# jpe17/TwoTowerMLRetrieval

Measured on AMD Instinct MI355X. Metric: queries/sec top-k over 10M x 256-d docs, higher is better.
Workload: dtype f32 results (bit-identical to the fp32 FMA chain); f16-MFMA screen + fp32 rescoring; 1 GPU; exact cosine top-10 of B=1024 queries over 10000000 x 256 fp32 unit-norm passages resident in HBM (BASELINE configs[3]; configs[1] batch), row-sharded over 1 GPU(s), screened path (f16-MFMA filter + exact fp32 rescoring, bit-identical to the fp32 kernel); n_docs=10000000, dim=256, batch=1024, k=10, parallelism=rowshard1

## Files before the change

### twotowermlretrieval_amd/csrc/screen.hip

```cpp
#include "score_topk.h"
#include "keep_word.h"
#include <cmath>

#include <hip/hip_fp16.h>
#include <limits.h>
#include <math.h>

namespace {

typedef _Float16 h8 __attribute__((ext_vector_type(8)));
typedef _Float16 h4 __attribute__((ext_vector_type(4)));
typedef unsigned u32x4 __attribute__((ext_vector_type(4)));
typedef __attribute__((address_space(3))) void lds_void;
typedef const __attribute__((address_space(1))) void gbl_void;

#ifndef TT_SCREEN_STAGGER
#define TT_SCREEN_STAGGER 1
#endif
constexpr int SW = 8;
constexpr int STILE_BYTES = 32 * 512;
constexpr int SRING = 8;
constexpr int STPB = 2;
constexpr int SCAP = 128;
constexpr int SURV_MAX = 1024;
constexpr int POOL_MAX = 8192;
constexpr int FIN_MAX_CHUNKS = 2048;

struct SCand {
    float v;
    int x;
};

__device__ __forceinline__ float screen_eps(float qnorm, float dmax)
{
    return 1.10e-3f * qnorm * dmax + 1e-6f * (qnorm + dmax);
}

template <int NCH>
__device__ __forceinline__ void bf16_to_f16_lds(char *base, int lane)
{
    uint4 v[NCH];
#pragma unroll
    for (int i = 0; i < NCH; ++i)
        v[i] = *(const uint4 *)(base + (i * 64 + lane) * 16);
#pragma unroll
    for (int i = 0; i < NCH; ++i) {
        unsigned w[4] = {v[i].x, v[i].y, v[i].z, v[i].w};
#pragma unroll
        for (int e = 0; e < 4; ++e) {
            const _Float16 lo = (_Float16)__uint_as_float(w[e] << 16);
            const _Float16 hi = (_Float16)__uint_as_float(w[e] & 0xffff0000u);
            w[e] = (unsigned)__builtin_bit_cast(unsigned short, lo) | ((unsigned)__builtin_bit_cast(unsigned short, hi) << 16);
        }
        *(uint4 *)(base + (i * 64 + lane) * 16) = uint4{w[0], w[1], w[2], w[3]};
    }
}

__device__ __forceinline__ SCand scand_load_l2(const SCand *p)
{
    unsigned long long u = __hip_atomic_load((const unsigned long long *)p, __ATOMIC_RELAXED, __HIP_MEMORY_SCOPE_AGENT);
    SCand c;
    c.v = __uint_as_float((unsigned)u);
    c.x = (int)(u >> 32);
    return c;
}

struct ScreenParams {
    const float *Q;
    const _Float16 *D16;
    int B, N, k;
    int n_chunks, tiles_per_chunk, n_tiles;
    int static_tiles, tail_g, tail_blocks;
    int *tail_ctr;
    float dmax;
    SCand *cand;
    int *pcnt;
    int *flag;
    float *max_val;
    const float *thr0;
    int thr0_stride;
    const h8 *qimg;
    const float *qnorm;
    const float *dbg_thr;
    const unsigned *keep;
};

__device__ __forceinline__ void scand_store_async(const SCand *base, unsigned byte_off, float v, int x)
{
    const unsigned long long bits = ((unsigned long long)(unsigned)x << 32) | (unsigned long long)__float_as_uint(v);
    asm volatile("global_store_dwordx2 %0, %1, %2\n\ts_nop 1" ::"v"(byte_off), "v"(bits), "s"(base) : "memory");
}

__device__ __forceinline__ void f32_store_async(float *dst, float v)
{
    asm volatile("global_store_dword %0, %1, off\n\ts_nop 0" ::"v"(dst), "v"(v) : "memory");
}

constexpr int SQUART = SCAP / 4;
constexpr int SQ_TRIGGER = SQUART - 10;
constexpr int SQ_KEEP_MAX = 4 * SQ_TRIGGER - 4;

__device__ __forceinline__ void screen_compact(SCand *base, const int (&n)[4], int k, float slack, int lane, int &n_new,
                                               float &thr_new, bool &have, bool &overflow)
{
    float v[2];
    int x[2], rank[2];
    bool live[2];
#pragma unroll
    for (int i = 0; i < 2; ++i) {
        v[i] = -INFINITY;
        x[i] = INT_MAX;
        rank[i] = 0;
        live[i] = (lane & 31) < ((lane >> 5) ? n[2 * i + 1] : n[2 * i]);
        if (live[i]) {
            const SCand c = scand_load_l2(base + 64 * i + lane);
            v[i] = c.v;
            x[i] = c.x;
        }
    }
#pragma unroll
    for (int i2 = 0; i2 < 2; ++i2) {
#pragma unroll
        for (int sub = 0; sub < 2; ++sub) {
            const int lim = n[2 * i2 + sub];
            for (int l2 = 0; l2 < lim; ++l2) {
                const float sv = __builtin_bit_cast(float, __builtin_amdgcn_readlane(__builtin_bit_cast(int, v[i2]), 32 * sub + l2));
                const int sx = __builtin_amdgcn_readlane(x[i2], 32 * sub + l2);
#pragma unroll
                for (int i = 0; i < 2; ++i)
                    rank[i] += (sv > v[i] || (sv == v[i] && sx < x[i])) ? 1 : 0;
            }
        }
    }
    const int total = n[0] + n[1] + n[2] + n[3];
    have = total >= k;
    overflow = false;
    n_new = total;
    thr_new = -INFINITY;
    if (have) {
        float kth = -INFINITY;
#pragma unroll
        for (int i = 0; i < 2; ++i) {
            const unsigned long long bk = __ballot(live[i] && rank[i] == k - 1);
            if (bk)
                kth = __builtin_bit_cast(float, __builtin_amdgcn_readlane(__builtin_bit_cast(int, v[i]), __ffsll((long long)bk) - 1));
        }
        thr_new = kth - slack;
        n_new = 0;
#pragma unroll
        for (int i = 0; i < 2; ++i)
            n_new += __popcll(__ballot(live[i] && v[i] >= thr_new));
        if (n_new > SQ_KEEP_MAX) {
            overflow = true;
            n_new = k;
        }
    }
#pragma unroll
    for (int i = 0; i < 2; ++i)
        if (live[i] && rank[i] < n_new) {
            SCand c;
            c.v = v[i];
            c.x = x[i];
            base[SQUART * (rank[i] & 3) + (rank[i] >> 2)] = c;
        }
}

__global__ __launch_bounds__(128) void q_image_kernel(const float *__restrict__ Q, int B, h8 *__restrict__ img,
                                                      float *__restrict__ qnorm, int *__restrict__ flag, int n_flags,
                                                      int *__restrict__ tail_ctr, int n_ctr)
{
    __shared__ int any_bad[2];
    if (blockIdx.x == 0)
        for (int i = threadIdx.x; i < n_ctr; i += 128)
            tail_ctr[i] = 0;
    const int lane = threadIdx.x & 63, wv = threadIdx.x >> 6;
    const int S = blockIdx.x * 2 + wv;
    const int g = lane >> 4, n = lane & 15;
    const int qrow = 16 * S + n;
    const bool live = qrow < B;
    const float *qp = Q + (size_t)min(qrow, B - 1) * 256 + 8 * g;
    float ss = 0.0f;
    bool bad = false;
#pragma unroll
    for (int s = 0; s < 8; ++s) {
        const f32x4 a = *(const f32x4 *)(qp + 32 * s);
        const f32x4 b = *(const f32x4 *)(qp + 32 * s + 4);
        h8 hv;
#pragma unroll
        for (int e = 0; e < 4; ++e) {
            const float x0 = live ? a[e] : 0.0f, x1 = live ? b[e] : 0.0f;
            ss += x0 * x0 + x1 * x1;
            bad |= !(fabsf(x0) <= 60000.0f) || !(fabsf(x1) <= 60000.0f);
            hv[e] = (_Float16)x0;
            hv[4 + e] = (_Float16)x1;
        }
        img[((size_t)S * 8 + s) * 64 + lane] = hv;
    }
    ss += __shfl_xor(ss, 16);
    ss += __shfl_xor(ss, 32);
    if (g == 0)
        qnorm[qrow] = sqrtf(ss);
    const bool wave_bad = __ballot(bad && live) != 0ull;
    if (lane == 0)
        any_bad[wv] = wave_bad ? 1 : 0;
    __syncthreads();
    if (threadIdx.x == 0 && (int)blockIdx.x < n_flags)
        flag[blockIdx.x] = (any_bad[0] | any_bad[1]) ? 2 : 0;
}

template <bool MAXONLY, int NSET, bool BF = false, bool MASKED = false>
__global__ __launch_bounds__(SW * 64, 2) void screen_kernel(ScreenParams p)
{
    extern __shared__ __attribute__((aligned(16))) char ring[];
    constexpr int DMA_AUX = NSET < 3 ? 2 : 0;
    const int lane = threadIdx.x & 63;
    const int w = __builtin_amdgcn_readfirstlane(threadIdx.x >> 6);
    const int chunk = blockIdx.x % p.n_chunks;
    const int qgroup = blockIdx.x / p.n_chunks;
    int t0 = chunk * p.tiles_per_chunk;
    int t1 = min(t0 + p.tiles_per_chunk, p.static_tiles);
    __shared__ int next_block;
    const int k = p.k;
    const int g = lane >> 4, n = lane & 15;
    constexpr int QW = 16 * NSET, QB = SW * QW;
    const int qbase = qgroup * QB + w * QW;
    const bool wave_live = qbase < p.B;

    h8 qreg[NSET][8];
    float eps2[NSET];
    f32x4 negthr[NSET];
    int cnt[NSET];
#pragma unroll
    for (int c = 0; c < NSET; ++c)
        cnt[c] = 0;
#pragma unroll
    for (int c = 0; c < NSET; ++c) {
        const int qrow = qbase + 16 * c + n;
        const bool live = qrow < p.B;
        float qn = 0.0f;
        if (wave_live) {
            const h8 *src = p.qimg + ((size_t)(qbase / 16 + c) * 8) * 64 + lane;
#pragma unroll
            for (int s = 0; s < 8; ++s)
                qreg[c][s] = src[s * 64];
            qn = p.qnorm[qrow];
        }
        eps2[c] = 2.0f * screen_eps(qn, p.dmax);
        const float floor_thr = -(1.01f * qn * p.dmax + 1e-30f);
        const float t_init = live ? ((!MAXONLY && p.thr0) ? fmaxf(p.thr0[(size_t)qrow * p.thr0_stride + p.thr0_stride - 1] - eps2[c], floor_thr)
                                                    : floor_thr)
                            : INFINITY;
        float c_init = -t_init;
        if (MAXONLY)
            c_init = (p.dbg_thr && live) ? -p.dbg_thr[qrow] : 0.0f;
        negthr[c] = f32x4{c_init, c_init, c_init, c_init};
    }

    SCand *const cwave = p.cand + ((size_t)blockIdx.x * QB + w * QW) * SCAP;

    auto compact_where = [&](int c, unsigned qmask) {
        asm volatile("s_waitcnt vmcnt(0)" ::: "memory");
        while (qmask) {
            const int q = __ffs((int)qmask) - 1;
            qmask &= qmask - 1;
            const int nq[4] = {__builtin_amdgcn_readlane(cnt[c], q), __builtin_amdgcn_readlane(cnt[c], q + 16),
                               __builtin_amdgcn_readlane(cnt[c], q + 32), __builtin_amdgcn_readlane(cnt[c], q + 48)};
            const float slack = __builtin_bit_cast(float, __builtin_amdgcn_readlane(__builtin_bit_cast(int, eps2[c]), q));
            int n_new;
            float tn;
            bool have, ovf;
            screen_compact(cwave + (size_t)(16 * c + q) * SCAP, nq, k, slack, lane, n_new, tn, have, ovf);
            if (ovf && lane == 0)
                atomicOr(p.flag + ((qbase + 16 * c) >> 5), 1);
            if (n == q) {
                cnt[c] = (n_new - g + 3) >> 2;
                if (have)
                    negthr[c] = f32x4{-tn, -tn, -tn, -tn};
            }
        }
    };

    const char *D = (const char *)p.D16;
    const char *rowp[2];
    auto set_rows = [&](int tile) {
#pragma unroll
        for (int i = 0; i < 2; ++i) {
            const int row = 2 * (2 * w + i) + (lane >> 5);
            const int doc = min(tile * 32 + row, p.N - 1);
            const int chunk16 = (lane & 31) ^ (row & 15);
            rowp[i] = D + (size_t)doc * 512 + chunk16 * 16;
        }
    };
    auto dma_issue = [&](int tile, int stage) {
        set_rows(min(tile, t1 - 1));
        char *dst = ring + stage * STILE_BYTES + (2 * w) * 1024;
        __builtin_amdgcn_global_load_lds((gbl_void *)rowp[0], (lds_void *)dst, 16, 0, DMA_AUX);
        __builtin_amdgcn_global_load_lds((gbl_void *)rowp[1], (lds_void *)(dst + 1024), 16, 0, DMA_AUX);
    };
    auto dma_piece = [&](int i, int stage) {
        char *dst = ring + stage * STILE_BYTES + (2 * w + i) * 1024;
        __builtin_amdgcn_global_load_lds((gbl_void *)rowp[i], (lds_void *)dst, 16, 0, DMA_AUX);
    };

    for (;;) {
    if (t0 < t1) {
#pragma unroll
        for (int gi = 0; gi < SRING - STPB; ++gi)
            dma_issue(t0 + gi, gi);
        int stage = 0;
        const int rd_base = n * 512;
        f32x4 acc[2][NSET];
        const bool late = TT_SCREEN_STAGGER && w >= 4;
        bool pending = false;
        int ptile = 0;
        unsigned pkw = 0xffffffffu;
        auto epilogue = [&](int tile, unsigned kw) {
                const int tile_base = tile * 32;
            const bool partial = tile_base + 32 > p.N;
            const bool holes = MASKED && kw != 0xffffffffu;
            const unsigned kwg = MASKED ? kw >> (4 * g) : 0xffffffffu;
            auto dropped = [&](int u, int r) {
                return tile_base + 16 * u + 4 * g + r >= p.N || (MASKED && ((kwg >> (16 * u + r)) & 1u) == 0u);
            };
            if (!MAXONLY) {
                if (partial || holes) {
#pragma unroll
                    for (int u = 0; u < 2; ++u)
#pragma unroll
                        for (int r = 0; r < 4; ++r)
                            if (dropped(u, r)) {
#pragma unroll
                                for (int c = 0; c < NSET; ++c)
                                    acc[u][c][r] = -INFINITY;
                            }
                }
                int mall = INT_MIN;
#pragma unroll
                for (int u = 0; u < 2; ++u)
#pragma unroll
                    for (int c = 0; c < NSET; ++c)
#pragma unroll
                        for (int r = 0; r < 4; ++r)
                            mall = max(mall, __float_as_int(acc[u][c][r]));
                if (__ballot(mall >= 0) != 0ull) {
#pragma unroll
                    for (int c = 0; c < NSET; ++c) {
                        int mu[2];
#pragma unroll
                        for (int u = 0; u < 2; ++u)
                            mu[u] = max(max(__float_as_int(acc[u][c][0]), __float_as_int(acc[u][c][1])),
                                        max(__float_as_int(acc[u][c][2]), __float_as_int(acc[u][c][3])));
                        if (__ballot(max(mu[0], mu[1]) >= 0) == 0ull)
                            continue;
                        const unsigned mine = (unsigned)(((16 * c + n) * SCAP + SQUART * g) * sizeof(SCand));
                        const float thr_c = -negthr[c][0];
#pragma unroll
                        for (int u = 0; u < 2; ++u) {
                            if (__ballot(mu[u] >= 0) == 0ull)
                                continue;
#pragma unroll
                            for (int r = 0; r < 4; ++r) {
                                if (__float_as_int(acc[u][c][r]) >= 0) {
                                    scand_store_async(cwave, mine + (unsigned)cnt[c] * (unsigned)sizeof(SCand),
                                                      acc[u][c][r] + thr_c, tile_base + 16 * u + 4 * g + r);
                                    ++cnt[c];
                                }
                            }
                        }
                        unsigned long long full = __ballot(cnt[c] > SQ_TRIGGER);
                        full = (full | (full >> 32));
                        full = (full | (full >> 16)) & 0xffffull;
                        if (full)
                            compact_where(c, (unsigned)full);
                    }
                }
            } else {
#pragma unroll
                for (int c = 0; c < NSET; ++c) {
                    float m = -INFINITY;
                    if (!partial && !holes) {
                        int mi = INT_MIN;
#pragma unroll
                        for (int u = 0; u < 2; ++u)
#pragma unroll
                            for (int r = 0; r < 4; ++r)
                                mi = max(mi, __float_as_int(acc[u][c][r]));
                        m = __int_as_float(mi);
                    } else {
#pragma unroll
                        for (int u = 0; u < 2; ++u)
#pragma unroll
                            for (int r = 0; r < 4; ++r)
                                m = fmaxf(m, !dropped(u, r) ? acc[u][c][r] : -INFINITY);
                    }
                    m = fmaxf(m, __shfl_xor(m, 16));
                    m = fmaxf(m, __shfl_xor(m, 32));
                    const int qrow = qbase + 16 * c + n;
                    if (g == 0 && qrow < p.B)
                        f32_store_async(p.max_val + (size_t)qrow * p.n_tiles + tile, m);
                }
            }
                };
        for (int tile = t0; tile < t1; ++tile) {
            if ((tile - t0) % STPB == 0) {
                asm volatile("s_waitcnt vmcnt(%0)" ::"n"(2 * (SRING - 2 * STPB)) : "memory");
                if (BF && tile == t0) {
#pragma unroll
                    for (int i = 0; i < STPB; ++i)
                        bf16_to_f16_lds<2>(ring + ((stage + i) % SRING) * STILE_BYTES + (2 * w) * 1024, lane);
                    asm volatile("s_waitcnt lgkmcnt(0)" ::: "memory");
                }
                __builtin_amdgcn_s_barrier();
            } else if (BF && (tile - t0) % STPB == STPB - 1) {
                asm volatile("s_waitcnt vmcnt(%0)" ::"n"(2 * (SRING - 3 * STPB + 1)) : "memory");
#pragma unroll
                for (int i = 1; i <= STPB; ++i)
                    bf16_to_f16_lds<2>(ring + ((stage + i) % SRING) * STILE_BYTES + (2 * w) * 1024, lane);
                asm volatile("s_waitcnt lgkmcnt(0)" ::: "memory");
            }
            const int fill_stage = (stage + SRING - STPB) % SRING;
            set_rows(min(tile + SRING - STPB, t1 - 1));
            if (!wave_live) {
                dma_piece(0, fill_stage);
                dma_piece(1, fill_stage);
            }
            if (wave_live) {
                if (late && pending)
                    epilogue(ptile, pkw);
                const char *buf = ring + stage * STILE_BYTES + rd_base;
                h8 a0[3], a1[3];
                auto a_read = [&](int s) {
                    const int off = ((4 * s + g) ^ n) << 4;
                    a0[s % 3] = *(const h8 *)(buf + off);
                    a1[s % 3] = *(const h8 *)(buf + 16 * 512 + off);
                };
                a_read(0);
                a_read(1);
                unsigned kw = 0xffffffffu;
#pragma unroll
                for (int s = 0; s < 8; ++s) {
                    if (s + 2 < 8)
                        a_read(s + 2);
                    if (MASKED && s == 0)
                        keep_word_issue(p.keep + __builtin_amdgcn_readfirstlane(tile), kw, a0[0]);
                    if (s == 2)
                        dma_piece(0, fill_stage);
                    if (s == 6)
                        dma_piece(1, fill_stage);
                    __builtin_amdgcn_sched_barrier(0);
#pragma unroll
                    for (int c = 0; c < NSET; ++c) {
                        const f32x4 c0 = s == 0 ? negthr[c] : acc[0][c];
                        const f32x4 c1 = s == 0 ? negthr[c] : acc[1][c];
                        acc[0][c] = __builtin_amdgcn_mfma_f32_16x16x32_f16(a0[s % 3], qreg[c][s], c0, 0, 0, 0);
                        acc[1][c] = __builtin_amdgcn_mfma_f32_16x16x32_f16(a1[s % 3], qreg[c][s], c1, 0, 0, 0);
                    }
                    __builtin_amdgcn_sched_barrier(0);
                }
                if (MASKED)
                    keep_word_wait(kw, acc[1][NSET - 1]);
                if (late) {
                    pending = true;
                    ptile = tile;
                    pkw = kw;
                } else {
                    epilogue(tile, kw);
                }
            }
            stage = (stage + 1) % SRING;
        }
        if (wave_live && late && pending)
            epilogue(ptile, pkw);
    }
    if (MAXONLY || p.tail_blocks == 0)
        break;
    asm volatile("s_waitcnt vmcnt(0)" ::: "memory");
    __builtin_amdgcn_s_barrier();
    if (threadIdx.x == 0)
        next_block = atomicAdd(p.tail_ctr + qgroup, 1);
    __syncthreads();
    const int blk = next_block;
    if (blk >= p.tail_blocks)
        break;
    t0 = p.static_tiles + blk * p.tail_g;
    t1 = min(t0 + p.tail_g, p.n_tiles);
    }
    asm volatile("s_waitcnt vmcnt(0)" ::: "memory");
    __builtin_amdgcn_s_barrier();

    if (MAXONLY)
        return;
#pragma unroll
    for (int c = 0; c < NSET; ++c) {
        int tot = cnt[c] + __shfl_xor(cnt[c], 16);
        tot += __shfl_xor(tot, 32);
        const unsigned long long over = __ballot(tot > k) & 0xffffull;
        if (over)
            compact_where(c, (unsigned)over);
        int packed = cnt[c] << (8 * g);
        packed |= __shfl_xor(packed, 16);
        packed |= __shfl_xor(packed, 32);
        const int qrow = qbase + 16 * c + n;
        if (g == 0 && qrow < p.B)
            p.pcnt[(size_t)qrow * p.n_chunks + chunk] = packed;
    }
}

constexpr int TW = 4;
constexpr int TSLAB_BYTES = 32 * 128;
constexpr int TSTAGE = 4;
constexpr int TDMA = 4;
constexpr int TSTREAM_AUX = 2;

template <bool MAXONLY, int NQS = 2, bool BF = false, bool MASKED = false>
__global__ __launch_bounds__(TW * 64, 2) void screen_stream_kernel(ScreenParams p)
{
    constexpr int QPT = 16 * NQS;
    extern __shared__ __attribute__((aligned(16))) char ring_all[];
    const int lane = threadIdx.x & 63;
    const int w = __builtin_amdgcn_readfirstlane(threadIdx.x >> 6);
    char *const ring = ring_all + w * (TSTAGE * TSLAB_BYTES);
    const int task = blockIdx.x * TW + w;
    const int n_qtiles = (p.B + QPT - 1) / QPT;
    if (task >= n_qtiles * p.n_chunks)
        return;
    const int qtile = task / p.n_chunks, chunk = task % p.n_chunks;
    const int t0 = chunk * p.tiles_per_chunk;
    const int t1 = min(t0 + p.tiles_per_chunk, p.n_tiles);
    const int k = p.k;
    const int g = lane >> 4, n = lane & 15;
    const int qbase = qtile * QPT;

    h8 qreg[NQS][8];
    float eps2[NQS];
    f32x4 negthr[NQS];
    int cnt[NQS];
#pragma unroll
    for (int c = 0; c < NQS; ++c) {
        cnt[c] = 0;
        const int qrow = qbase + 16 * c + n;
        const bool live = qrow < p.B;
        const h8 *src = p.qimg + ((size_t)(qbase / 16 + c) * 8) * 64 + lane;
#pragma unroll
        for (int s = 0; s < 8; ++s)
            qreg[c][s] = src[s * 64];
        const float qn = p.qnorm[qrow];
        eps2[c] = 2.0f * screen_eps(qn, p.dmax);
        const float floor_thr = -(1.01f * qn * p.dmax + 1e-30f);
        const float t_init = live ? ((!MAXONLY && p.thr0) ? fmaxf(p.thr0[(size_t)qrow * p.thr0_stride + p.thr0_stride - 1] - eps2[c], floor_thr)
                                                    : floor_thr)
                            : INFINITY;
        float c_init = -t_init;
        if (MAXONLY)
            c_init = (p.dbg_thr && live) ? -p.dbg_thr[qrow] : 0.0f;
        negthr[c] = f32x4{c_init, c_init, c_init, c_init};
    }

    SCand *const cwave = p.cand + (size_t)task * QPT * SCAP;

    auto compact_where = [&](int c, unsigned qmask) {
        asm volatile("s_waitcnt vmcnt(0)" ::: "memory");
        while (qmask) {
            const int q = __ffs((int)qmask) - 1;
            qmask &= qmask - 1;
            const int nq[4] = {__builtin_amdgcn_readlane(cnt[c], q), __builtin_amdgcn_readlane(cnt[c], q + 16),
                               __builtin_amdgcn_readlane(cnt[c], q + 32), __builtin_amdgcn_readlane(cnt[c], q + 48)};
            const float slack = __builtin_bit_cast(float, __builtin_amdgcn_readlane(__builtin_bit_cast(int, eps2[c]), q));
            int n_new;
            float tn;
            bool have, ovf;
            screen_compact(cwave + (size_t)(16 * c + q) * SCAP, nq, k, slack, lane, n_new, tn, have, ovf);
            if (ovf && lane == 0)
                atomicOr(p.flag + ((qbase + 16 * c) >> 5), 1);
            if (n == q) {
                cnt[c] = (n_new - g + 3) >> 2;
                if (have)
                    negthr[c] = f32x4{-tn, -tn, -tn, -tn};
            }
        }
    };

    const char *D = (const char *)p.D16;
    int dma_tile = t0, dma_kq = 0;
    const char *rowp[TDMA];
    auto set_rows = [&](int tile) {
#pragma unroll
        for (int jj = 0; jj < TDMA; ++jj) {
            const int row = 8 * jj + (lane >> 3);
            const int doc = min(tile * 32 + row, p.N - 1);
            rowp[jj] = D + (size_t)doc * 512 + (((lane & 7) ^ (row & 7)) << 4);
        }
    };
    auto dma_issue = [&](int stage) {
        char *dst = ring + stage * TSLAB_BYTES;
#pragma unroll
        for (int jj = 0; jj < TDMA; ++jj)
            __builtin_amdgcn_global_load_lds((gbl_void *)(rowp[jj] + dma_kq * 128), (lds_void *)(dst + jj * 1024), 16, 0, TSTREAM_AUX);
        if (++dma_kq == 4) {
            dma_kq = 0;
            dma_tile = min(dma_tile + 1, t1 - 1);
            set_rows(dma_tile);
        }
    };

    if (t0 < t1) {
        set_rows(t0);
#pragma unroll
        for (int i = 0; i < TSTAGE - 1; ++i)
            dma_issue(i);
        int stage = 0;
        const char *rd_row = ring + n * 128;
        const int rsw = n & 7;
        for (int tile = t0; tile < t1; ++tile) {
            f32x4 acc[2][NQS];
            unsigned kw = 0xffffffffu;
#pragma unroll
            for (int kq = 0; kq < 4; ++kq) {
                asm volatile("s_waitcnt vmcnt(%0)" ::"n"(TDMA * (TSTAGE - 2)) : "memory");
                if (BF) {
                    bf16_to_f16_lds<TSLAB_BYTES / 1024>(ring + stage * TSLAB_BYTES, lane);
                    asm volatile("s_waitcnt lgkmcnt(0)" ::: "memory");
                }
                const char *buf = rd_row + stage * TSLAB_BYTES;
                h8 a[2][2];
#pragma unroll
                for (int s2 = 0; s2 < 2; ++s2)
#pragma unroll
                    for (int u = 0; u < 2; ++u)
                        a[u][s2] = *(const h8 *)(buf + u * 2048 + (((4 * s2 + g) ^ rsw) << 4));
                asm volatile("s_waitcnt lgkmcnt(0)" ::: "memory");
                if (MASKED && kq == 3)
                    keep_word_issue(p.keep + tile, kw, a[0][0]);
                dma_issue((stage + TSTAGE - 1) % TSTAGE);
#pragma unroll
                for (int s2 = 0; s2 < 2; ++s2)
#pragma unroll
                    for (int c = 0; c < NQS; ++c)
#pragma unroll
                        for (int u = 0; u < 2; ++u) {
                            const f32x4 cin = (kq == 0 && s2 == 0) ? negthr[c] : acc[u][c];
                            acc[u][c] = __builtin_amdgcn_mfma_f32_16x16x32_f16(a[u][s2], qreg[c][2 * kq + s2], cin, 0, 0, 0);
                        }
                stage = (stage + 1) % TSTAGE;
            }
            const int tile_base = tile * 32;
            const bool partial = tile_base + 32 > p.N;
            if (MASKED)
                keep_word_wait(kw, acc[1][NQS - 1]);
            const bool holes = MASKED && kw != 0xffffffffu;
            const unsigned kwg = MASKED ? kw >> (4 * g) : 0xffffffffu;
            auto dropped = [&](int u, int r) {
                return tile_base + 16 * u + 4 * g + r >= p.N || (MASKED && ((kwg >> (16 * u + r)) & 1u) == 0u);
            };
            if (!MAXONLY) {
                if (MASKED && kw == 0u)
                    continue;
                if (partial || holes) {
#pragma unroll
                    for (int u = 0; u < 2; ++u)
#pragma unroll
                        for (int r = 0; r < 4; ++r)
                            if (dropped(u, r)) {
#pragma unroll
                                for (int c = 0; c < NQS; ++c)
                                    acc[u][c][r] = -INFINITY;
                            }
                }
                int mall = INT_MIN;
#pragma unroll
                for (int u = 0; u < 2; ++u)
#pragma unroll
                    for (int c = 0; c < NQS; ++c)
#pragma unroll
                        for (int r = 0; r < 4; ++r)
                            mall = max(mall, __float_as_int(acc[u][c][r]));
                if (__ballot(mall >= 0) != 0ull) {
#pragma unroll
                    for (int c = 0; c < NQS; ++c) {
                        const unsigned mine = (unsigned)(((16 * c + n) * SCAP + SQUART * g) * sizeof(SCand));
                        const float thr_c = -negthr[c][0];
#pragma unroll
                        for (int u = 0; u < 2; ++u)
#pragma unroll
                            for (int r = 0; r < 4; ++r) {
                                if (__float_as_int(acc[u][c][r]) >= 0) {
                                    scand_store_async(cwave, mine + (unsigned)cnt[c] * (unsigned)sizeof(SCand),
                                                      acc[u][c][r] + thr_c, tile_base + 16 * u + 4 * g + r);
                                    ++cnt[c];
                                }
                            }
                        unsigned long long full = __ballot(cnt[c] > SQ_TRIGGER);
                        full = (full | (full >> 32));
                        full = (full | (full >> 16)) & 0xffffull;
                        if (full)
                            compact_where(c, (unsigned)full);
                    }
                }
            } else {
#pragma unroll
                for (int c = 0; c < NQS; ++c) {
                    float m = -INFINITY;
#pragma unroll
                    for (int u = 0; u < 2; ++u)
#pragma unroll
                        for (int r = 0; r < 4; ++r)
                            m = fmaxf(m, ((!partial && !holes) || !dropped(u, r)) ? acc[u][c][r] : -INFINITY);
                    m = fmaxf(m, __shfl_xor(m, 16));
                    m = fmaxf(m, __shfl_xor(m, 32));
                    const int qrow = qbase + 16 * c + n;
                    if (g == 0 && qrow < p.B)
                        f32_store_async(p.max_val + (size_t)qrow * p.n_tiles + tile, m);
                }
            }
        }
    }
    asm volatile("s_waitcnt vmcnt(0)" ::: "memory");
    if (MAXONLY)
        return;
#pragma unroll
    for (int c = 0; c < NQS; ++c) {
        int tot = cnt[c] + __shfl_xor(cnt[c], 16);
        tot += __shfl_xor(tot, 32);
        const unsigned long long over = __ballot(tot > k) & 0xffffull;
        if (over)
            compact_where(c, (unsigned)over);
        int packed = cnt[c] << (8 * g);
        packed |= __shfl_xor(packed, 16);
        packed |= __shfl_xor(packed, 32);
        const int qrow = qbase + 16 * c + n;
        if (g == 0 && qrow < p.B)
            p.pcnt[(size_t)qrow * p.n_chunks + chunk] = packed;
    }
}

struct FinishParams {
    const float *Q;
    const float *D32;
    const unsigned *Dbf;
    int B, N, k, n_chunks;
    float dmax;
    const SCand *cand;
    const int *pcnt;
    int *flag;
    int64_t idx_offset;
    float *out_val;
    int64_t *out_idx;
    int q_per_block;
    int *stats;
};

__device__ __forceinline__ bool before_f(float sa, int ia, float sb, int ib) { return sa > sb || (sa == sb && ia < ib); }

__device__ __forceinline__ unsigned f32_order_key(float f)
{
    const unsigned b = __float_as_uint(f);
    return (b & 0x80000000u) ? ~b : (b | 0x80000000u);
}
__device__ __forceinline__ float f32_from_order_key(unsigned k)
{
    return __uint_as_float((k & 0x80000000u) ? (k & 0x7fffffffu) : ~k);
}

__global__ __launch_bounds__(256) void screen_finish_kernel(FinishParams p)
{
    __shared__ float pool_v[POOL_MAX];
    __shared__ float qs[256];
    __shared__ float sv_v[SURV_MAX];
    __shared__ int sv_x[SURV_MAX];
    __shared__ float red_v[4];
    __shared__ int hist[256];
    extern __shared__ int fin_dyn[];
    int *const ccnt = fin_dyn;
    int *const pre = fin_dyn + p.n_chunks;
    __shared__ int sel[2];
    __shared__ int n_pool, n_surv;
    const int row = blockIdx.x, tid = threadIdx.x;
    if (tid == 0)
        n_pool = n_surv = 0;
    qs[tid] = p.Q[(size_t)row * 256 + tid];
    __syncthreads();
    float ss = qs[tid] * qs[tid];
#pragma unroll
    for (int off = 32; off >= 1; off >>= 1)
        ss += __shfl_xor(ss, off);
    if ((tid & 63) == 0)
        red_v[tid >> 6] = ss;
    __syncthreads();
    const float eps2 = 2.0f * screen_eps(sqrtf(red_v[0] + red_v[1] + red_v[2] + red_v[3]), p.dmax);
    __syncthreads();
// ... 825 lines not shown
```

Baseline: 260,300 queries/s.

## Use buffer-load LDS DMA, interleave MFMA with LDS reads, raise late-wave priority

Replaces the per-lane global_load_lds row pointers with buffer_load_dwordx4 ... lds, using a scalar resource descriptor set once per tile and precomputed per-lane offsets. This removes the per-tile 64-bit address arithmetic and VGPR pressure. It also interleaves the A-fragment LDS reads and the DMA issues between individual MFMAs, and raises the scheduling priority of the staggered late waves. The changes depend on hand-written m0 save/restore inline asm and sched barriers, which is fragile and could hurt if issue ordering or descriptor bounds are wrong.

```diff
diff --git a/twotowermlretrieval_amd/csrc/screen.hip b/twotowermlretrieval_amd/csrc/screen.hip
--- a/twotowermlretrieval_amd/csrc/screen.hip
+++ b/twotowermlretrieval_amd/csrc/screen.hip
@@ -16,6 +16,15 @@
 
 #ifndef TT_SCREEN_STAGGER
 #define TT_SCREEN_STAGGER 1
+#endif
+#ifndef TT_SCREEN_BUFDMA
+#define TT_SCREEN_BUFDMA 1
+#endif
+#ifndef TT_SCREEN_INTERLEAVE
+#define TT_SCREEN_INTERLEAVE 1
+#endif
+#ifndef TT_SCREEN_PRIO
+#define TT_SCREEN_PRIO 1
 #endif
 constexpr int SW = 8;
 constexpr int STILE_BYTES = 32 * 512;
@@ -118,6 +127,7 @@
             x[i] = c.x;
         }
     }
+    asm volatile("" : "+v"(v[0]), "+v"(x[0]), "+v"(v[1]), "+v"(x[1]));
 #pragma unroll
     for (int i2 = 0; i2 < 2; ++i2) {
 #pragma unroll
@@ -244,6 +254,11 @@
             for (int s = 0; s < 8; ++s)
                 qreg[c][s] = src[s * 64];
             qn = p.qnorm[qrow];
+#if TT_SCREEN_BUFDMA
+#pragma unroll
+            for (int s = 0; s < 8; ++s)
+                asm volatile("" : "+v"(qreg[c][s]));
+#endif
         }
         eps2[c] = 2.0f * screen_eps(qn, p.dmax);
         const float floor_thr = -(1.01f * qn * p.dmax + 1e-30f);
@@ -281,6 +296,43 @@
     };
 
     const char *D = (const char *)p.D16;
+#if TT_SCREEN_BUFDMA
+    const unsigned ring_lds = __builtin_amdgcn_readfirstlane((unsigned)(size_t)(lds_void *)ring);
+    unsigned voff[2];
+#pragma unroll
+    for (int i = 0; i < 2; ++i) {
+        const int row = 2 * (2 * w + i) + (lane >> 5);
+        voff[i] = (unsigned)(row * 512 + ((((lane & 31) ^ (row & 15))) << 4));
+    }
+    const unsigned long long d_bytes = (unsigned long long)p.N * 512ull;
+    u32x4 rsrc;
+    auto set_rows = [&](int tile) {
+        const unsigned long long off = (unsigned long long)(unsigned)__builtin_amdgcn_readfirstlane(tile) * (unsigned long long)STILE_BYTES;
+        const unsigned long long base = (unsigned long long)(size_t)D + off;
+        const unsigned long long left = d_bytes - off;
+        rsrc[0] = (unsigned)base;
+        rsrc[1] = (unsigned)(base >> 32) & 0xffffu;
+        rsrc[2] = (unsigned)(left >> 32) ? 0xffffffffu : (unsigned)left;
+        rsrc[3] = 0x00020000u;
+    };
+    auto dma_piece = [&](int i, int stage) {
+        const unsigned dst = ring_lds + (unsigned)(stage * STILE_BYTES + (2 * w + i) * 1024);
+        unsigned m0_keep;
+        if (DMA_AUX == 2)
+            asm volatile("s_nop 4\n\ts_mov_b32 %0, m0\n\ts_mov_b32 m0, %3\n\ts_nop 0\n\t"
+                         "buffer_load_dwordx4 %1, %2, 0 offen nt lds\n\ts_mov_b32 m0, %0"
+                         : "=&s"(m0_keep) : "v"(voff[i]), "s"(rsrc), "s"(dst) : "memory");
+        else
+            asm volatile("s_nop 4\n\ts_mov_b32 %0, m0\n\ts_mov_b32 m0, %3\n\ts_nop 0\n\t"
+                         "buffer_load_dwordx4 %1, %2, 0 offen lds\n\ts_mov_b32 m0, %0"
+                         : "=&s"(m0_keep) : "v"(voff[i]), "s"(rsrc), "s"(dst) : "memory");
+    };
+    auto dma_issue = [&](int tile, int stage) {
+        set_rows(min(tile, t1 - 1));
+        dma_piece(0, stage);
+        dma_piece(1, stage);
+    };
+#else
     const char *rowp[2];
     auto set_rows = [&](int tile) {
 #pragma unroll
@@ -301,6 +353,10 @@
         char *dst = ring + stage * STILE_BYTES + (2 * w + i) * 1024;
         __builtin_amdgcn_global_load_lds((gbl_void *)rowp[i], (lds_void *)dst, 16, 0, DMA_AUX);
     };
+#endif
+
+    if (TT_SCREEN_PRIO && w >= 4)
+        __builtin_amdgcn_s_setprio(1);
 
     for (;;) {
     if (t0 < t1) {
@@ -437,6 +493,30 @@
                 a_read(0);
                 a_read(1);
                 unsigned kw = 0xffffffffu;
+#if TT_SCREEN_INTERLEAVE
+#pragma unroll
+                for (int s = 0; s < 8; ++s) {
+                    if (MASKED && s == 0)
+                        keep_word_issue(p.keep + __builtin_amdgcn_readfirstlane(tile), kw, a0[0]);
+#pragma unroll
+                    for (int j = 0; j < 2 * NSET; ++j) {
+                        const int c = j >> 1, u = j & 1;
+                        const f32x4 cin = s == 0 ? negthr[c] : acc[u][c];
+                        acc[u][c] = __builtin_amdgcn_mfma_f32_16x16x32_f16(u ? a1[s % 3] : a0[s % 3], qreg[c][s], cin, 0, 0, 0);
+                        __builtin_amdgcn_sched_barrier(0);
+                        if (s + 2 < 8 && j < 2) {
+                            const int off = ((4 * (s + 2) + g) ^ n) << 4;
+                            if (j == 0)
+                                a0[(s + 2) % 3] = *(const h8 *)(buf + off);
+                            else
+                                a1[(s + 2) % 3] = *(const h8 *)(buf + 16 * 512 + off);
+                        }
+                        if (NSET >= 2 ? (j == 2 && (s == 2 || s == 6)) : (j == 0 && s >= 6))
+                            dma_piece(NSET >= 2 ? s / 6 : s - 6, fill_stage);
+                        __builtin_amdgcn_sched_barrier(0);
+                    }
+                }
+#else
 #pragma unroll
                 for (int s = 0; s < 8; ++s) {
                     if (s + 2 < 8)
@@ -457,6 +537,7 @@
                     }
                     __builtin_amdgcn_sched_barrier(0);
                 }
+#endif
                 if (MASKED)
                     keep_word_wait(kw, acc[1][NSET - 1]);
                 if (late) {
@@ -485,6 +566,8 @@
     t0 = p.static_tiles + blk * p.tail_g;
     t1 = min(t0 + p.tail_g, p.n_tiles);
     }
+    if (TT_SCREEN_PRIO)
+        __builtin_amdgcn_s_setprio(0);
     asm volatile("s_waitcnt vmcnt(0)" ::: "memory");
     __builtin_amdgcn_s_barrier();
 
```

Result: no change. 260,200 queries/s (-0.1%).
